# nirschl-lab/stain2stain

Hardware: AMD Instinct MI355X
Metric: paired 256x256 stain tiles/sec (full CFM optimisation step) (higher is better)
Workload: dtype bf16

## Files before the change

stain2stain_amd/csrc/conv3x3_wgrad_mfma.hip:

```cpp
#include "common.h"
#include <stdlib.h>
#include <type_traits>

struct WgradArgs {
  const void* dy;
  const void* x0;
  const void* x1;
  float* part;
  int lddy, Cout, ld0, c0, ld1, c1;
  int B, H, W, tilesY, tilesX, ntiles, S;
  int lgc;
  int lgh, lgw;
  int xcd;
};

namespace {

template <typename T> struct WPiece;
template <> struct WPiece<bf16_t> {
  bf16x8 v;
  __device__ __forceinline__ void zero() {
#pragma unroll
    for (int i = 0; i < 8; ++i) v[i] = (bf16_t)0.0f;
  }
  __device__ __forceinline__ void load(const bf16_t* p) { v = *reinterpret_cast<const bf16x8*>(p); }
  __device__ __forceinline__ void to_lds(char* hi, int, int off) const { *reinterpret_cast<bf16x8*>(hi + off) = v; }
};
template <> struct WPiece<float> {
  f32x4 a, b;
  __device__ __forceinline__ void zero() {
#pragma unroll
    for (int i = 0; i < 4; ++i) { a[i] = 0.f; b[i] = 0.f; }
  }
  __device__ __forceinline__ void load(const float* p) {
    a = *reinterpret_cast<const f32x4*>(p);
    b = *reinterpret_cast<const f32x4*>(p + 4);
  }
  __device__ __forceinline__ void to_lds(char* hi, int img_stride, int off) const {
    bf16x8 h, m, l;
#pragma unroll
    for (int i = 0; i < 8; ++i) {
      const float x = i < 4 ? a[i] : b[i - 4];
      h[i] = (bf16_t)x;
      const float r1 = x - (float)h[i];
      m[i] = (bf16_t)r1;
      l[i] = (bf16_t)(r1 - (float)m[i]);
    }
    *reinterpret_cast<bf16x8*>(hi + off) = h;
    *reinterpret_cast<bf16x8*>(hi + img_stride + off) = m;
    *reinterpret_cast<bf16x8*>(hi + 2 * img_stride + off) = l;
  }
};

typedef __attribute__((address_space(3))) s16x4 lds_s16x4;

__device__ __forceinline__ bf16x8 tr_frag(const char* p_rows0, int row_stride4) {
  s16x4 lo = __builtin_amdgcn_ds_read_tr16_b64_v4i16((lds_s16x4*)(p_rows0));
  s16x4 hi = __builtin_amdgcn_ds_read_tr16_b64_v4i16((lds_s16x4*)(p_rows0 + row_stride4));
  bf16x4 l4 = __builtin_bit_cast(bf16x4, lo), h4 = __builtin_bit_cast(bf16x4, hi);
  bf16x8 r;
#pragma unroll
  for (int i = 0; i < 4; ++i) { r[i] = l4[i]; r[4 + i] = h4[i]; }
  return r;
}

template <typename T, int TH, int TW>
__global__ __launch_bounds__(256, (std::is_same<T, float>::value ? 1 : 2)) void conv3x3_wgrad_kernel(WgradArgs a) {
  constexpr bool SPLIT = std::is_same<T, float>::value;
  constexpr int NIMG = SPLIT ? 3 : 1;
  constexpr int NPX = TH * TW;
  constexpr int HW_ = TW + 2, HALO = (TH + 2) * HW_;
  constexpr int DY_BYTES = 2 * NPX * 64;
  constexpr int X_BYTES = 2 * HALO * 64;
  constexpr int DY_PIECES = NPX * 8, DY_IT = (DY_PIECES + 255) / 256;
  constexpr int X_PIECES = HALO * 8, X_IT = (X_PIECES + 255) / 256;
  constexpr int KSTEPS = NPX / 16;
  static_assert(TW % 16 == 0, "a k-step is 16 consecutive pixels of one tile row");

  extern __shared__ __attribute__((aligned(16))) char smem[];
  char* const ldsDY = smem;
  char* const ldsX = smem + NIMG * DY_BYTES;

  const T* __restrict__ dy = static_cast<const T*>(a.dy);
  const T* __restrict__ x0 = static_cast<const T*>(a.x0);
  const T* __restrict__ x1 = static_cast<const T*>(a.x1);

  const int tid = threadIdx.x, lane = tid & 63, wave = tid >> 6;
  const int wco = wave >> 1, wci = wave & 1;
  const int ci0 = blockIdx.x * 64, co0 = blockIdx.y * 64;
  const int cin = a.c0 + a.c1;

  const int g = lane >> 4, q = (lane & 15) >> 2, p = lane & 3;
  const int frag_off = ((g >> 1) * 8 + q) * 64 + ((g & 1) * 16 + p * 4) * 2;

  f32x16 acc[9];
#pragma unroll
  for (int t = 0; t < 9; ++t)
#pragma unroll
    for (int j = 0; j < 16; ++j) acc[t][j] = 0.f;

  WPiece<T> dreg[DY_IT];
  WPiece<T> xreg[X_IT];

  auto load_tile = [&](int tile) {
    int bt = tile;
    const int tx = bt % a.tilesX; bt /= a.tilesX;
    const int ty = bt % a.tilesY;
    const int img = bt / a.tilesY;
    const int y0 = ty * TH, xs = tx * TW;
#pragma unroll
    for (int i = 0; i < DY_IT; ++i) {
      const int idx = tid + i * 256;
      const int px = idx >> 3, pc = idx & 7;
      const int py = px / TW, pxx = px - py * TW;
      const int gy = y0 + py, gx = xs + pxx, co = co0 + pc * 8;
      dreg[i].zero();
      if (idx < DY_PIECES && gy < a.H && gx < a.W && co < a.Cout)
        dreg[i].load(dy + ((long)(img * a.H + gy) * a.W + gx) * a.lddy + co);
    }
#pragma unroll
    for (int i = 0; i < X_IT; ++i) {
      const int idx = tid + i * 256;
      const int px = idx >> 3, pc = idx & 7;
      const int hy = px / HW_, hx = px - hy * HW_;
      const int gy = y0 - 1 + hy, gx = xs - 1 + hx, ci = ci0 + pc * 8;
      xreg[i].zero();
      if (idx < X_PIECES && gy >= 0 && gy < a.H && gx >= 0 && gx < a.W) {
        const long pix = (long)(img * a.H + gy) * a.W + gx;
        if (ci < a.c0) xreg[i].load(x0 + pix * a.ld0 + ci);
        else if (ci < cin) xreg[i].load(x1 + pix * a.ld1 + (ci - a.c0));
      }
    }
  };
  auto store_tile = [&]() {
#pragma unroll
    for (int i = 0; i < DY_IT; ++i) {
      const int idx = tid + i * 256;
      const int px = idx >> 3, pc = idx & 7;
      if (idx < DY_PIECES)
        dreg[i].to_lds(ldsDY, DY_BYTES, (pc >> 2) * (NPX * 64) + px * 64 + (pc & 3) * 16);
    }
#pragma unroll
    for (int i = 0; i < X_IT; ++i) {
      const int idx = tid + i * 256;
      const int px = idx >> 3, pc = idx & 7;
      if (idx < X_PIECES)
        xreg[i].to_lds(ldsX, X_BYTES, (pc >> 2) * (HALO * 64) + px * 64 + (pc & 3) * 16);
    }
  };

  const char* const Ahi = ldsDY + wco * (NPX * 64) + frag_off;
  const char* const Bhi = ldsX + wci * (HALO * 64) + frag_off;

  int tile = blockIdx.z;
  if (tile < a.ntiles) load_tile(tile);
  for (; tile < a.ntiles; tile += a.S) {
    __syncthreads();
    store_tile();
    __syncthreads();
    if (tile + a.S < a.ntiles) load_tile(tile + a.S);
#pragma unroll
    for (int ks = 0; ks < KSTEPS; ++ks) {
      const int m0 = ks * 16;
      const int py = m0 / TW, px = m0 - py * TW;
      const bf16x8 af = tr_frag(Ahi + m0 * 64, 4 * 64);
      bf16x8 am, al;
      if constexpr (SPLIT) {
        am = tr_frag(Ahi + DY_BYTES + m0 * 64, 4 * 64);
        al = tr_frag(Ahi + 2 * DY_BYTES + m0 * 64, 4 * 64);
      }
#pragma unroll
      for (int tap = 0; tap < 9; ++tap) {
        const int hoff = ((py + tap / 3) * HW_ + px + tap % 3) * 64;
        const bf16x8 bfr = tr_frag(Bhi + hoff, 4 * 64);
        if constexpr (SPLIT) {
          const bf16x8 bm = tr_frag(Bhi + X_BYTES + hoff, 4 * 64);
          const bf16x8 bl = tr_frag(Bhi + 2 * X_BYTES + hoff, 4 * 64);
          acc[tap] = __builtin_amdgcn_mfma_f32_32x32x16_bf16(am, bm, acc[tap], 0, 0, 0);
          acc[tap] = __builtin_amdgcn_mfma_f32_32x32x16_bf16(al, bfr, acc[tap], 0, 0, 0);
          acc[tap] = __builtin_amdgcn_mfma_f32_32x32x16_bf16(af, bl, acc[tap], 0, 0, 0);
          acc[tap] = __builtin_amdgcn_mfma_f32_32x32x16_bf16(am, bfr, acc[tap], 0, 0, 0);
          acc[tap] = __builtin_amdgcn_mfma_f32_32x32x16_bf16(af, bm, acc[tap], 0, 0, 0);
        }
        acc[tap] = __builtin_amdgcn_mfma_f32_32x32x16_bf16(af, bfr, acc[tap], 0, 0, 0);
      }
    }
  }

  const int r = lane & 31, h = lane >> 5;
  const int ci = ci0 + wci * 32 + r;
#pragma unroll
  for (int tap = 0; tap < 9; ++tap) {
#pragma unroll
    for (int j = 0; j < 16; ++j) {
      const int co = co0 + wco * 32 + (j & 3) + 8 * (j >> 2) + 4 * h;
      if (co < a.Cout && ci < cin)
        a.part[(((long)blockIdx.z * 9 + tap) * a.Cout + co) * cin + ci] = acc[tap][j];
    }
  }
}

__device__ __attribute__((aligned(64))) char g_wgrad_zero_page[64];
typedef __attribute__((address_space(3))) void lds_void_t;
typedef __attribute__((address_space(1))) const void gbl_void_t;

__device__ __forceinline__ void dma16_asm(const void* gsrc, unsigned lds_dst) {
  unsigned keep;
  asm volatile("s_mov_b32 %0, m0\n\ts_mov_b32 m0, %2\n\ts_nop 0\n\tglobal_load_lds_dwordx4 %1, off\n\ts_mov_b32 m0, %0"
               : "=&s"(keep) : "v"(gsrc), "s"(lds_dst) : "memory");
}

template <int TH, int TW>
__global__ __launch_bounds__(256, 2) void conv3x3_wgrad_dma_kernel(WgradArgs a) {
  using T = bf16_t;
  constexpr int NW = 4, NT = 9;
  constexpr int NPX = TH * TW;
  constexpr int HW_ = TW + 2, HR = TH + 2, HALO = HR * HW_;
  constexpr int XROWS = (HALO + 31) / 32 * 32;
  constexpr int DY_BYTES = 2 * NPX * 64, X_BYTES = 2 * XROWS * 64;
  constexpr int DYGRP = 2 * NPX / 16, XGRP = 2 * XROWS / 16;
  constexpr int DYG = DYGRP / NW;
  constexpr int XG = XGRP / NW;
  constexpr int BUF = DY_BYTES + X_BYTES;
  constexpr int KSTEPS = NPX / 16;
  static_assert(DYGRP % 4 == 0 && XGRP % 4 == 0, "DMA groups split evenly over 4 waves");

  extern __shared__ __attribute__((aligned(16))) char smem[];
  const T* __restrict__ dy = static_cast<const T*>(a.dy);
  const T* __restrict__ x0 = static_cast<const T*>(a.x0);
  const T* __restrict__ x1 = static_cast<const T*>(a.x1);

  const int tid = threadIdx.x, lane = tid & 63;
  const int wave = __builtin_amdgcn_readfirstlane(tid >> 6);
  const int wco = (wave & 3) >> 1, wci = wave & 1;
  unsigned bx = blockIdx.x, by = blockIdx.y, bz = blockIdx.z;
  if (a.xcd) {
    const unsigned L = bx + gridDim.x * (by + gridDim.y * bz), per = gridDim.x * gridDim.y * gridDim.z / 8;
    unsigned Lq = (L & 7) * per + (L >> 3);
    bx = Lq % gridDim.x; Lq /= gridDim.x;
    by = Lq % gridDim.y; bz = Lq / gridDim.y;
  }
  const int ci0 = bx * 64, co0 = by * 64;
  const int cin = a.c0 + a.c1;
  const int drow = lane >> 2, dslot = lane & 3;
  const int zsplit = (int)bz;

  const int g = lane >> 4, q = (lane & 15) >> 2, p = lane & 3;
  const int frag_off = ((g >> 1) * 8 + q) * 64 + ((g & 1) * 16 + p * 4) * 2;

  f32x16 acc[NT];
#pragma unroll
  for (int t = 0; t < NT; ++t)
#pragma unroll
    for (int j = 0; j < 16; ++j) acc[t][j] = 0.f;

  int dy_off[DYG], dy_py[DYG], dy_px[DYG];
  bool dy_ok[DYG];
#pragma unroll
  for (int j = 0; j < DYG; ++j) {
    const int grp = wave + NW * j;
    const int half = grp / (NPX / 16), px = (grp % (NPX / 16)) * 16 + drow;
    const int co = co0 + half * 32 + dslot * 8;
    dy_py[j] = px / TW; dy_px[j] = px - dy_py[j] * TW;
    dy_ok[j] = co < a.Cout;
    dy_off[j] = (dy_py[j] * a.W + dy_px[j]) * a.lddy + co;
  }
  const T* x_ptr[XG];
  int x_off[XG], x_ld[XG], x_hy[XG], x_hx[XG];
#pragma unroll
  for (int j = 0; j < XG; ++j) {
    const int grp = wave + NW * j;
    const int half = grp / (XROWS / 16), px = (grp % (XROWS / 16)) * 16 + drow;
    const int ci = ci0 + half * 32 + dslot * 8;
    x_hy[j] = px / HW_; x_hx[j] = px - x_hy[j] * HW_;
    x_ptr[j] = nullptr; x_ld[j] = 0;
    if (px < HALO) {
      if (ci < a.c0) { x_ptr[j] = x0 + ci; x_ld[j] = a.ld0; }
      else if (ci < cin) { x_ptr[j] = x1 + (ci - a.c0); x_ld[j] = a.ld1; }
    }
    x_off[j] = ((x_hy[j] - 1) * a.W + (x_hx[j] - 1)) * x_ld[j];
  }

  auto dma_tile = [&](int tile, int buf) {
    int bt = tile;
    const int tx = bt % a.tilesX; bt /= a.tilesX;
    const int ty = bt % a.tilesY;
    const int img = bt / a.tilesY;
    const int y0 = ty * TH, xs = tx * TW;
    const long pixbase = (long)(img * a.H + y0) * a.W + xs;
    const bool interior = y0 >= 1 && y0 + TH + 1 <= a.H && xs >= 1 && xs + TW + 1 <= a.W;
    const unsigned base = (unsigned)(uintptr_t)(__attribute__((address_space(3))) char*)smem + buf * BUF;
    if (interior) {
#pragma unroll
      for (int j = 0; j < DYG; ++j) {
        const void* src = dy_ok[j] ? (const void*)(dy + pixbase * a.lddy + dy_off[j]) : (const void*)g_wgrad_zero_page;
        dma16_asm(src, __builtin_amdgcn_readfirstlane(base + (wave + NW * j) * 1024));
      }
#pragma unroll
      for (int j = 0; j < XG; ++j) {
        const void* src = x_ptr[j] ? (const void*)(x_ptr[j] + pixbase * x_ld[j] + x_off[j]) : (const void*)g_wgrad_zero_page;
        dma16_asm(src, __builtin_amdgcn_readfirstlane(base + DY_BYTES + (wave + NW * j) * 1024));
      }
    } else {
#pragma unroll
      for (int j = 0; j < DYG; ++j) {
        const int gy = y0 + dy_py[j], gx = xs + dy_px[j];
        const void* src = g_wgrad_zero_page;
        if (gy < a.H && gx < a.W && dy_ok[j]) src = dy + pixbase * a.lddy + dy_off[j];
        dma16_asm(src, __builtin_amdgcn_readfirstlane(base + (wave + NW * j) * 1024));
      }
#pragma unroll
      for (int j = 0; j < XG; ++j) {
        const int gy = y0 - 1 + x_hy[j], gx = xs - 1 + x_hx[j];
        const void* src = g_wgrad_zero_page;
        if (x_ptr[j] && gy >= 0 && gy < a.H && gx >= 0 && gx < a.W) src = x_ptr[j] + pixbase * x_ld[j] + x_off[j];
        dma16_asm(src, __builtin_amdgcn_readfirstlane(base + DY_BYTES + (wave + NW * j) * 1024));
      }
    }
  };

  int tile = zsplit;
  int buf = 0;
  if (tile < a.ntiles) dma_tile(tile, 0);
  asm volatile("s_waitcnt vmcnt(0)" ::: "memory");
  __builtin_amdgcn_s_barrier();
  for (; tile < a.ntiles; tile += a.S) {
    if (tile + a.S < a.ntiles) dma_tile(tile + a.S, buf ^ 1);
    const char* const Ahi = smem + buf * BUF + wco * (NPX * 64) + frag_off;
    const char* const Bhi = smem + buf * BUF + DY_BYTES + wci * (XROWS * 64) + frag_off;
#pragma unroll
    for (int ks = 0; ks < KSTEPS; ++ks) {
      const int m0 = ks * 16;
      const int py = m0 / TW, px = m0 - py * TW;
      const bf16x8 af = tr_frag(Ahi + m0 * 64, 4 * 64);
#pragma unroll
      for (int t = 0; t < NT; ++t) {
        const int hoff = ((py + t / 3) * HW_ + px + t % 3) * 64;
        const bf16x8 bfr = tr_frag(Bhi + hoff, 4 * 64);
        acc[t] = __builtin_amdgcn_mfma_f32_32x32x16_bf16(af, bfr, acc[t], 0, 0, 0);
      }
    }
    __builtin_amdgcn_sched_barrier(0);
    asm volatile("s_waitcnt vmcnt(0)" ::: "memory");
    __builtin_amdgcn_s_barrier();
    buf ^= 1;
  }

  const int r = lane & 31, h = lane >> 5;
  const int ci = ci0 + wci * 32 + r;
#pragma unroll
  for (int t = 0; t < NT; ++t) {
#pragma unroll
    for (int j = 0; j < 16; ++j) {
      const int co = co0 + wco * 32 + (j & 3) + 8 * (j >> 2) + 4 * h;
      if (co < a.Cout && ci < cin)
        a.part[(((long)zsplit * 9 + t) * a.Cout + co) * cin + ci] = acc[t][j];
    }
  }
}

template <int ZG>
__global__ __launch_bounds__(64 * ZG) void wgrad_reduce_kernel(const float* __restrict__ part, float* __restrict__ grad, int S, int Cout,
                                    int Cin, int accumulate) {
  __shared__ float tile[ZG][9][65];
  const long n = (long)Cout * Cin;
  const int il = threadIdx.x & 63, zg = threadIdx.x >> 6;
  const long i = (long)blockIdx.x * 64 + il;
  float s[9];
#pragma unroll
  for (int t = 0; t < 9; ++t) s[t] = 0.f;
  if (i < n) {
    for (int z = zg; z < S; z += ZG)
#pragma unroll
      for (int t = 0; t < 9; ++t) s[t] += part[((long)z * 9 + t) * n + i];
  }
#pragma unroll
  for (int t = 0; t < 9; ++t) tile[zg][t][il] = s[t];
  __syncthreads();
  const long base = (long)blockIdx.x * 64 * 9;
  for (int k = threadIdx.x; k < 576; k += 64 * ZG) {
    const long o = base + k;
    if (o < n * 9) {
      const int t = k % 9, j = k / 9;
      float v = 0.f;
#pragma unroll
      for (int g = 0; g < ZG; g += 4) v += (tile[g][t][j] + tile[g + 1][t][j]) + (tile[g + 2][t][j] + tile[g + 3][t][j]);
      grad[o] = accumulate ? grad[o] + v : v;
    }
  }
}

template <typename T, int TH, int TW>
int launch_wgrad(WgradArgs& a, hipStream_t s) {
  constexpr int NIMG = std::is_same<T, float>::value ? 3 : 1;
  constexpr int lds = NIMG * (2 * TH * TW * 64 + 2 * (TH + 2) * (TW + 2) * 64);
  a.tilesY = cdiv(a.H, TH);
  a.tilesX = cdiv(a.W, TW);
  a.ntiles = a.B * a.tilesY * a.tilesX;
  if (a.S > a.ntiles) return S2S_ERR_SHAPE;
  auto kern = conv3x3_wgrad_kernel<T, TH, TW>;
  static unsigned long long attr_devs = 0;
  if (int rc = s2s_allow_dyn_lds(reinterpret_cast<const void*>(kern), lds, &attr_devs)) return rc;
  dim3 grid(cdiv(a.c0 + a.c1, 64), cdiv(a.Cout, 64), a.S);
  hipLaunchKernelGGL(kern, grid, dim3(256), lds, s, a);
  S2S_LAUNCH_CHECK();
  return S2S_OK;
}

template <int TH, int TW>
int launch_wgrad_dma(WgradArgs& a, hipStream_t s) {
  constexpr int XROWS = ((TH + 2) * (TW + 2) + 31) / 32 * 32;
  constexpr int lds = 2 * (2 * TH * TW * 64 + 2 * XROWS * 64);
  a.tilesY = cdiv(a.H, TH);
  a.tilesX = cdiv(a.W, TW);
  a.ntiles = a.B * a.tilesY * a.tilesX;
  if (a.S > a.ntiles) return S2S_ERR_SHAPE;
  auto kern = conv3x3_wgrad_dma_kernel<TH, TW>;
  static unsigned long long attr_devs = 0;
  if (int rc = s2s_allow_dyn_lds(reinterpret_cast<const void*>(kern), lds, &attr_devs)) return rc;
  dim3 grid(cdiv(a.c0 + a.c1, 64), cdiv(a.Cout, 64), a.S);
  static const int xcd_aware = [] { const char* e = getenv("S2S_WGRAD_XCD"); return e ? atoi(e) : 1; }();
  a.xcd = xcd_aware && ((long)grid.x * grid.y * grid.z) % 8 == 0;
  hipLaunchKernelGGL(kern, grid, dim3(256), lds, s, a);
  S2S_LAUNCH_CHECK();
  return S2S_OK;
}

template <int TH, int TW, bool S2D = false>
__global__ __launch_bounds__(256, 2) void conv2x2_wgrad_dma_kernel(WgradArgs a) {
  using T = bf16_t;
  constexpr int NT = 4;
  constexpr int NPX = TH * TW;
  constexpr int HW_ = TW + 1, HR = TH + 1, HALO = HR * HW_;
  constexpr int XROWS = (HALO + 31) / 32 * 32;
  constexpr int DY_BYTES = 2 * NPX * 64, X_BYTES = 2 * XROWS * 64;
  constexpr int DYG = 2 * NPX / 16 / 4;
  constexpr int XG = 2 * XROWS / 16 / 4;
  constexpr int BUF = DY_BYTES + X_BYTES;
  constexpr int KSTEPS = NPX / 16;
  static_assert((2 * NPX / 16) % 4 == 0 && (2 * XROWS / 16) % 4 == 0, "DMA groups split evenly over 4 waves");

  extern __shared__ __attribute__((aligned(16))) char smem[];
  const T* __restrict__ dy = static_cast<const T*>(a.dy);
  const T* __restrict__ x0 = static_cast<const T*>(a.x0);

  const int tid = threadIdx.x, lane = tid & 63;
  const int wave = __builtin_amdgcn_readfirstlane(tid >> 6);
  const int wco = wave >> 1, wci = wave & 1;
  const int ci0 = blockIdx.x * 64, co0 = blockIdx.y * 64;
  const int cin = a.c0;
  const int Hi = a.H + 1, Wi = a.W + 1;
  const int drow = lane >> 2, dslot = lane & 3;
  const int zsplit = (int)blockIdx.z;

  const int g = lane >> 4, q = (lane & 15) >> 2, p = lane & 3;
  const int frag_off = ((g >> 1) * 8 + q) * 64 + ((g & 1) * 16 + p * 4) * 2;

  f32x16 acc[NT];
#pragma unroll
  for (int t = 0; t < NT; ++t)
#pragma unroll
    for (int j = 0; j < 16; ++j) acc[t][j] = 0.f;

  int dy_off[DYG], dy_py[DYG], dy_px[DYG];
  bool dy_ok[DYG];
#pragma unroll
  for (int j = 0; j < DYG; ++j) {
    const int grp = wave + 4 * j;
    const int half = grp / (NPX / 16), px = (grp % (NPX / 16)) * 16 + drow;
    const int co = co0 + half * 32 + dslot * 8;
    dy_py[j] = px / TW; dy_px[j] = px - dy_py[j] * TW;
    dy_ok[j] = co < a.Cout;
    dy_off[j] = (dy_py[j] * a.W + dy_px[j]) * a.lddy + co;
  }
  const T* x_ptr[XG];
  int x_off[XG], x_hy[XG], x_hx[XG];
#pragma unroll
  for (int j = 0; j < XG; ++j) {
    const int grp = wave + 4 * j;
    const int half = grp / (XROWS / 16), px = (grp % (XROWS / 16)) * 16 + drow;
    const int ci = ci0 + half * 32 + dslot * 8;
    x_hy[j] = px / HW_; x_hx[j] = px - x_hy[j] * HW_;
    if (S2D) {
      const int rs = ci >> a.lgc;
      x_ptr[j] = (px < HALO && ci < cin) ? x0 + (ci & ((1 << a.lgc) - 1)) : nullptr;
      x_hy[j] = 2 * x_hy[j] + (rs >> 1) - 1;
      x_hx[j] = 2 * x_hx[j] + (rs & 1) - 1;
      x_off[j] = 0;
    } else {
      x_ptr[j] = (px < HALO && ci < cin) ? x0 + ci : nullptr;
      x_off[j] = (x_hy[j] * Wi + x_hx[j]) * a.ld0;
    }
  }

  auto dma_tile = [&](int tile, int buf) {
    int bt = tile;
    const int tx = bt % a.tilesX; bt /= a.tilesX;
    const int ty = bt % a.tilesY;
    const int img = bt / a.tilesY;
    const int y0 = ty * TH, xs = tx * TW;
    const long pixbase = (long)(img * a.H + y0) * a.W + xs;
    const long xbase = (long)(img * Hi + y0) * Wi + xs;
    const bool interior = !S2D && y0 + TH <= a.H && xs + TW <= a.W;
    const unsigned base = (unsigned)(uintptr_t)(__attribute__((address_space(3))) char*)smem + buf * BUF;
    if (interior) {
#pragma unroll
      for (int j = 0; j < DYG; ++j) {
        const void* src = dy_ok[j] ? (const void*)(dy + pixbase * a.lddy + dy_off[j]) : (const void*)g_wgrad_zero_page;
        dma16_asm(src, __builtin_amdgcn_readfirstlane(base + (wave + 4 * j) * 1024));
      }
#pragma unroll
      for (int j = 0; j < XG; ++j) {
        const void* src = x_ptr[j] ? (const void*)(x_ptr[j] + xbase * a.ld0 + x_off[j]) : (const void*)g_wgrad_zero_page;
        dma16_asm(src, __builtin_amdgcn_readfirstlane(base + DY_BYTES + (wave + 4 * j) * 1024));
      }
    } else {
#pragma unroll
      for (int j = 0; j < DYG; ++j) {
        const int gy = y0 + dy_py[j], gx = xs + dy_px[j];
        const void* src = g_wgrad_zero_page;
        if (gy < a.H && gx < a.W && dy_ok[j]) src = dy + pixbase * a.lddy + dy_off[j];
        dma16_asm(src, __builtin_amdgcn_readfirstlane(base + (wave + 4 * j) * 1024));
      }
#pragma unroll
      for (int j = 0; j < XG; ++j) {
        const void* src = g_wgrad_zero_page;
        if (S2D) {
          const int py = 2 * y0 + x_hy[j], px = 2 * xs + x_hx[j];
          if (x_ptr[j] && (unsigned)py < (unsigned)(2 * a.H) && (unsigned)px < (unsigned)(2 * a.W))
            src = x_ptr[j] + ((long)(img * 2 * a.H + py) * (2 * a.W) + px) * a.ld0;
        } else {
          const int gy = y0 + x_hy[j], gx = xs + x_hx[j];
          if (x_ptr[j] && gy < Hi && gx < Wi) src = x_ptr[j] + xbase * a.ld0 + x_off[j];
        }
        dma16_asm(src, __builtin_amdgcn_readfirstlane(base + DY_BYTES + (wave + 4 * j) * 1024));
      }
    }
  };

  int tile = zsplit;
  int buf = 0;
  if (tile < a.ntiles) dma_tile(tile, 0);
  asm volatile("s_waitcnt vmcnt(0)" ::: "memory");
  __builtin_amdgcn_s_barrier();
  for (; tile < a.ntiles; tile += a.S) {
    if (tile + a.S < a.ntiles) dma_tile(tile + a.S, buf ^ 1);
    const char* const Ahi = smem + buf * BUF + wco * (NPX * 64) + frag_off;
    const char* const Bhi = smem + buf * BUF + DY_BYTES + wci * (XROWS * 64) + frag_off;
#pragma unroll
    for (int ks = 0; ks < KSTEPS; ++ks) {
      const int m0 = ks * 16;
      const int py = m0 / TW, px = m0 - py * TW;
      const bf16x8 af = tr_frag(Ahi + m0 * 64, 4 * 64);
#pragma unroll
      for (int t = 0; t < NT; ++t) {
        const int hoff = ((py + t / 2) * HW_ + px + t % 2) * 64;
        const bf16x8 bfr = tr_frag(Bhi + hoff, 4 * 64);
        acc[t] = __builtin_amdgcn_mfma_f32_32x32x16_bf16(af, bfr, acc[t], 0, 0, 0);
      }
    }
    __builtin_amdgcn_sched_barrier(0);
    asm volatile("s_waitcnt vmcnt(0)" ::: "memory");
    __builtin_amdgcn_s_barrier();
    buf ^= 1;
  }

  const int r = lane & 31, h = lane >> 5;
  const int ci = ci0 + wci * 32 + r;
#pragma unroll
  for (int t = 0; t < NT; ++t) {
#pragma unroll
    for (int j = 0; j < 16; ++j) {
      const int co = co0 + wco * 32 + (j & 3) + 8 * (j >> 2) + 4 * h;
      if (co < a.Cout && ci < cin)
        a.part[(((long)zsplit * NT + t) * a.Cout + co) * cin + ci] = acc[t][j];
    }
  }
}

__global__ __launch_bounds__(256, 1) void conv2x2_wgrad_flat_kernel(WgradArgs a) {
  using T = bf16_t;
  constexpr int NT = 4, NPX = 128;
  constexpr int DY_BYTES = 2 * NPX * 64, PLANE = NPX * 64, X_BYTES = 2 * NT * PLANE;
  constexpr int DYG = 2 * NPX / 16 / 4;
  constexpr int XG = 2 * NT * NPX / 16 / 4;
  constexpr int KSTEPS = NPX / 16;

  extern __shared__ __attribute__((aligned(16))) char smem[];
  const T* __restrict__ dy = static_cast<const T*>(a.dy);
  const T* __restrict__ x0 = static_cast<const T*>(a.x0);
  const int tid = threadIdx.x, lane = tid & 63;
  const int wave = __builtin_amdgcn_readfirstlane(tid >> 6);
  const int wco = wave >> 1, wci = wave & 1;
  const int ci0 = blockIdx.x * 64, co0 = blockIdx.y * 64;
  const int cin = a.c0;
  const int h = 1 << a.lgh, w = 1 << a.lgw;
  const int npix = a.B << (a.lgh + a.lgw);
  const int drow = lane >> 2, dslot = lane & 3;
  const int zsplit = (int)blockIdx.z;
  const int g = lane >> 4, q = (lane & 15) >> 2, p4 = lane & 3;
  const int frag_off = ((g >> 1) * 8 + q) * 64 + ((g & 1) * 16 + p4 * 4) * 2;

  f32x16 acc[NT];
#pragma unroll
  for (int t = 0; t < NT; ++t)
#pragma unroll
    for (int j = 0; j < 16; ++j) acc[t][j] = 0.f;

  auto dma_tile = [&](int tile) {
    const int p0 = tile * NPX;
    const unsigned base = (unsigned)(uintptr_t)(__attribute__((address_space(3))) char*)smem;
#pragma unroll
    for (int j = 0; j < DYG; ++j) {
      const int grp = wave + 4 * j;
      const int half = grp / (NPX / 16), m = (grp % (NPX / 16)) * 16 + drow;
      const int co = co0 + half * 32 + dslot * 8, p = p0 + m;
      const void* src = g_wgrad_zero_page;
      if (p < npix && co < a.Cout) src = dy + (long)p * a.lddy + co;
      dma16_asm(src, __builtin_amdgcn_readfirstlane(base + grp * 1024));
    }
#pragma unroll
    for (int j = 0; j < XG; ++j) {
      const int grp = wave + 4 * j;
      const int half = grp >> 5, tap = (grp >> 3) & 3, m = (grp & 7) * 16 + drow;
      const int ci = ci0 + half * 32 + dslot * 8, p = p0 + m;
      const void* src = g_wgrad_zero_page;
      if (p < npix && ci < cin) {
        const int n = p >> (a.lgh + a.lgw), iy = (p >> a.lgw) & (h - 1), ix = p & (w - 1);
        const int rs = ci >> a.lgc, cc = ci & ((1 << a.lgc) - 1);
        const int py = 2 * (iy + (tap >> 1)) + (rs >> 1) - 1, px = 2 * (ix + (tap & 1)) + (rs & 1) - 1;
        if ((unsigned)py < (unsigned)(2 * h) && (unsigned)px < (unsigned)(2 * w))
          src = x0 + ((long)(n * 2 * h + py) * (2 * w) + px) * a.ld0 + cc;
      }
      dma16_asm(src, __builtin_amdgcn_readfirstlane(base + DY_BYTES + grp * 1024));
    }
  };

  for (int tile = zsplit; tile < a.ntiles; tile += a.S) {
    dma_tile(tile);
    asm volatile("s_waitcnt vmcnt(0)" ::: "memory");
    __builtin_amdgcn_s_barrier();
    const char* const Ahi = smem + wco * (NPX * 64) + frag_off;
    const char* const Bhi = smem + DY_BYTES + wci * (NT * PLANE) + frag_off;
#pragma unroll
    for (int ks = 0; ks < KSTEPS; ++ks) {
      const int m0 = ks * 16;
      const bf16x8 af = tr_frag(Ahi + m0 * 64, 4 * 64);
#pragma unroll
      for (int t = 0; t < NT; ++t) {
        const bf16x8 bfr = tr_frag(Bhi + t * PLANE + m0 * 64, 4 * 64);
        acc[t] = __builtin_amdgcn_mfma_f32_32x32x16_bf16(af, bfr, acc[t], 0, 0, 0);
      }
    }
    __builtin_amdgcn_sched_barrier(0);
    asm volatile("s_waitcnt lgkmcnt(0)" ::: "memory");
    __builtin_amdgcn_s_barrier();
  }
  const int r = lane & 31, hh = lane >> 5;
  const int ci = ci0 + wci * 32 + r;
#pragma unroll
  for (int t = 0; t < NT; ++t) {
#pragma unroll
    for (int j = 0; j < 16; ++j) {
      const int co = co0 + wco * 32 + (j & 3) + 8 * (j >> 2) + 4 * hh;
      if (co < a.Cout && ci < cin) a.part[(((long)zsplit * NT + t) * a.Cout + co) * cin + ci] = acc[t][j];
    }
  }
}

__global__ __launch_bounds__(256, 2) void conv2x2_wgrad_small_kernel(WgradArgs a, float* __restrict__ grad, int accumulate) {
  using T = bf16_t;
  constexpr int NT = 4, NPX = 128;
  constexpr int DY_BYTES = 2 * NPX * 64, PLANE = NPX * 64, X_BYTES = 2 * NT * PLANE, BUF = DY_BYTES + X_BYTES;
  constexpr int DYG = 2 * NPX / 16 / 4;
  constexpr int XG = 2 * NT * NPX / 16 / 4;
  constexpr int KSTEPS = NPX / 16;

  extern __shared__ __attribute__((aligned(16))) char smem[];
  const T* __restrict__ dy = static_cast<const T*>(a.dy);
  const T* __restrict__ x0 = static_cast<const T*>(a.x0);
  const int tid = threadIdx.x, lane = tid & 63;
  const int wave = __builtin_amdgcn_readfirstlane(tid >> 6);
  const int wco = wave >> 1, wci = wave & 1;
  const int c0 = blockIdx.x * 16, co0 = blockIdx.y * 64;
  const int C = a.c0 >> 2;
  const int h = 1 << a.lgh, w = 1 << a.lgw;
  const int npix = a.B << (a.lgh + a.lgw);
  const int drow = lane >> 2, dslot = lane & 3;
  const int g = lane >> 4, q = (lane & 15) >> 2, p4 = lane & 3;
  const int frag_off = ((g >> 1) * 8 + q) * 64 + ((g & 1) * 16 + p4 * 4) * 2;

  f32x16 acc[NT];
#pragma unroll
  for (int t = 0; t < NT; ++t)
#pragma unroll
    for (int j = 0; j < 16; ++j) acc[t][j] = 0.f;

  auto dma_tile = [&](int tile, int buf) {
    const int p0 = tile * NPX;
    const unsigned base = (unsigned)(uintptr_t)(__attribute__((address_space(3))) char*)smem + buf * BUF;
#pragma unroll
    for (int j = 0; j < DYG; ++j) {
      const int grp = wave + 4 * j;
      const int half = grp / (NPX / 16), m = (grp % (NPX / 16)) * 16 + drow;
      const int co = co0 + half * 32 + dslot * 8, p = p0 + m;
      const void* src = g_wgrad_zero_page;
      if (p < npix && co < a.Cout) src = dy + (long)p * a.lddy + co;
      dma16_asm(src, __builtin_amdgcn_readfirstlane(base + grp * 1024));
    }
#pragma unroll
    for (int j = 0; j < XG; ++j) {
      const int grp = wave + 4 * j;
      const int half = grp >> 5, tap = (grp >> 3) & 3, m = (grp & 7) * 16 + drow;
      const int vci = half * 32 + dslot * 8, rs = vci >> 4, cc = c0 + (vci & 15), p = p0 + m;
      const void* src = g_wgrad_zero_page;
      if (p < npix && cc < C) {
        const int n = p >> (a.lgh + a.lgw), iy = (p >> a.lgw) & (h - 1), ix = p & (w - 1);
        const int py = 2 * (iy + (tap >> 1)) + (rs >> 1) - 1, px = 2 * (ix + (tap & 1)) + (rs & 1) - 1;
        if ((unsigned)py < (unsigned)(2 * h) && (unsigned)px < (unsigned)(2 * w))
          src = x0 + ((long)(n * 2 * h + py) * (2 * w) + px) * a.ld0 + cc;
      }
      dma16_asm(src, __builtin_amdgcn_readfirstlane(base + DY_BYTES + grp * 1024));
// ... 623 lines not shown
```

Measured before the change: 2262.

## Use buffer-load LDS DMA with OOB zeroing and interleave prefetch with MFMA k-steps

Swaps global_load_lds plus a zero-page pointer select for buffer_load...lds with per-tile buffer resource descriptors, so out-of-bounds halo and channel lanes are zero-filled by hardware range checking instead of branchy address selection. The next tile's DMA pieces are now spread across the k-step loop, two per step, instead of being issued in one burst before compute. Halo B fragments are reused across k-steps through a rolling 3x3 register window, which cuts repeated LDS transposed reads. It adds a shape guard on the descriptor's record range, a MIXED template variant for concat inputs whose split is not 32-aligned, and ablation variants behind a compile flag.

```diff
diff --git a/stain2stain_amd/csrc/conv3x3_wgrad_mfma.hip b/stain2stain_amd/csrc/conv3x3_wgrad_mfma.hip
--- a/stain2stain_amd/csrc/conv3x3_wgrad_mfma.hip
+++ b/stain2stain_amd/csrc/conv3x3_wgrad_mfma.hip
@@ -1,6 +1,7 @@
 #include "common.h"
 #include <stdlib.h>
 #include <type_traits>
+
 
 struct WgradArgs {
   const void* dy;
@@ -210,9 +211,25 @@
                : "=&s"(keep) : "v"(gsrc), "s"(lds_dst) : "memory");
 }
 
-template <int TH, int TW>
+typedef __attribute__((ext_vector_type(4))) int i32x4;
+constexpr unsigned WG_RECORDS = 0x80000000u;
+constexpr unsigned WG_OOB = 0xffffff00u;
+__device__ __forceinline__ i32x4 wgrad_rsrc(uintptr_t base) {
+  i32x4 r;
+  r[0] = __builtin_amdgcn_readfirstlane((int)(unsigned)base);
+  r[1] = __builtin_amdgcn_readfirstlane((int)((base >> 32) & 0xffff));
+  r[2] = (int)WG_RECORDS;
+  r[3] = 0x00020000;
+  return r;
+}
+__device__ __forceinline__ void dma16_buf(const i32x4& rsrc, unsigned voff, unsigned lds_dst) {
+  unsigned keep;
+  asm volatile("s_mov_b32 %0, m0\n\ts_mov_b32 m0, %3\n\ts_nop 0\n\tbuffer_load_dwordx4 %1, %2, 0 offen lds\n\ts_mov_b32 m0, %0"
+               : "=&s"(keep) : "v"(voff), "s"(rsrc), "s"(lds_dst));
+}
+
+template <int TH, int TW, bool MIXED, int ABL>
 __global__ __launch_bounds__(256, 2) void conv3x3_wgrad_dma_kernel(WgradArgs a) {
-  using T = bf16_t;
   constexpr int NW = 4, NT = 9;
   constexpr int NPX = TH * TW;
   constexpr int HW_ = TW + 2, HR = TH + 2, HALO = HR * HW_;
@@ -221,15 +238,15 @@
   constexpr int DYGRP = 2 * NPX / 16, XGRP = 2 * XROWS / 16;
   constexpr int DYG = DYGRP / NW;
   constexpr int XG = XGRP / NW;
+  constexpr int NP = DYG + XG;
   constexpr int BUF = DY_BYTES + X_BYTES;
   constexpr int KSTEPS = NPX / 16;
   static_assert(DYGRP % 4 == 0 && XGRP % 4 == 0, "DMA groups split evenly over 4 waves");
+  constexpr int PK = (NP + 1) / 2;
+  static_assert(PK < KSTEPS, "pieces land before the tile-end wait");
+  static_assert(TW == 16, "a k-step is one tile row");
 
   extern __shared__ __attribute__((aligned(16))) char smem[];
-  const T* __restrict__ dy = static_cast<const T*>(a.dy);
-  const T* __restrict__ x0 = static_cast<const T*>(a.x0);
-  const T* __restrict__ x1 = static_cast<const T*>(a.x1);
-
   const int tid = threadIdx.x, lane = tid & 63;
   const int wave = __builtin_amdgcn_readfirstlane(tid >> 6);
   const int wco = (wave & 3) >> 1, wci = wave & 1;
@@ -254,96 +271,114 @@
 #pragma unroll
     for (int j = 0; j < 16; ++j) acc[t][j] = 0.f;
 
-  int dy_off[DYG], dy_py[DYG], dy_px[DYG];
-  bool dy_ok[DYG];
+  unsigned dy_voff[DYG];
+  int dy_py[DYG], dy_px[DYG];
 #pragma unroll
   for (int j = 0; j < DYG; ++j) {
     const int grp = wave + NW * j;
     const int half = grp / (NPX / 16), px = (grp % (NPX / 16)) * 16 + drow;
     const int co = co0 + half * 32 + dslot * 8;
     dy_py[j] = px / TW; dy_px[j] = px - dy_py[j] * TW;
-    dy_ok[j] = co < a.Cout;
-    dy_off[j] = (dy_py[j] * a.W + dy_px[j]) * a.lddy + co;
-  }
-  const T* x_ptr[XG];
-  int x_off[XG], x_ld[XG], x_hy[XG], x_hx[XG];
+    dy_voff[j] = co < a.Cout ? (unsigned)(((dy_py[j] * a.W + dy_px[j]) * a.lddy + co) * 2) : WG_OOB;
+  }
+  unsigned x_voff[XG];
+  int x_hy[XG], x_hx[XG], x_mode[XG];
+  bool x_hi[XG];
 #pragma unroll
   for (int j = 0; j < XG; ++j) {
     const int grp = wave + NW * j;
     const int half = grp / (XROWS / 16), px = (grp % (XROWS / 16)) * 16 + drow;
-    const int ci = ci0 + half * 32 + dslot * 8;
+    const int cbase = ci0 + half * 32, ci = cbase + dslot * 8;
     x_hy[j] = px / HW_; x_hx[j] = px - x_hy[j] * HW_;
-    x_ptr[j] = nullptr; x_ld[j] = 0;
-    if (px < HALO) {
-      if (ci < a.c0) { x_ptr[j] = x0 + ci; x_ld[j] = a.ld0; }
-      else if (ci < cin) { x_ptr[j] = x1 + (ci - a.c0); x_ld[j] = a.ld1; }
-    }
-    x_off[j] = ((x_hy[j] - 1) * a.W + (x_hx[j] - 1)) * x_ld[j];
-  }
-
-  auto dma_tile = [&](int tile, int buf) {
+    x_mode[j] = __builtin_amdgcn_readfirstlane(cbase + 32 <= a.c0 || a.c1 == 0 ? 0 : cbase >= a.c0 ? 1 : 2);
+    x_hi[j] = ci >= a.c0;
+    const int ld = x_hi[j] ? a.ld1 : a.ld0, ch = x_hi[j] ? ci - a.c0 : ci;
+    x_voff[j] = px < HALO && ci < cin ? (unsigned)(((x_hy[j] * a.W + x_hx[j]) * ld + ch) * 2) : WG_OOB;
+  }
+
+  struct TileSrc {
+    i32x4 rdy, rx0, rx1;
+    int limy, limx, sy, sx;
+  };
+  auto tile_src = [&](int tile) {
     int bt = tile;
     const int tx = bt % a.tilesX; bt /= a.tilesX;
     const int ty = bt % a.tilesY;
     const int img = bt / a.tilesY;
     const int y0 = ty * TH, xs = tx * TW;
-    const long pixbase = (long)(img * a.H + y0) * a.W + xs;
-    const bool interior = y0 >= 1 && y0 + TH + 1 <= a.H && xs >= 1 && xs + TW + 1 <= a.W;
-    const unsigned base = (unsigned)(uintptr_t)(__attribute__((address_space(3))) char*)smem + buf * BUF;
-    if (interior) {
-#pragma unroll
-      for (int j = 0; j < DYG; ++j) {
-        const void* src = dy_ok[j] ? (const void*)(dy + pixbase * a.lddy + dy_off[j]) : (const void*)g_wgrad_zero_page;
-        dma16_asm(src, __builtin_amdgcn_readfirstlane(base + (wave + NW * j) * 1024));
-      }
-#pragma unroll
-      for (int j = 0; j < XG; ++j) {
-        const void* src = x_ptr[j] ? (const void*)(x_ptr[j] + pixbase * x_ld[j] + x_off[j]) : (const void*)g_wgrad_zero_page;
-        dma16_asm(src, __builtin_amdgcn_readfirstlane(base + DY_BYTES + (wave + NW * j) * 1024));
-      }
+    const long pix = (long)(img * a.H + y0) * a.W + xs;
+    const long hpix = pix - a.W - 1;
+    TileSrc s;
+    s.rdy = wgrad_rsrc((uintptr_t)a.dy + (uintptr_t)(pix * a.lddy * 2));
+    s.rx0 = wgrad_rsrc((uintptr_t)a.x0 + (uintptr_t)(hpix * a.ld0 * 2));
+    s.rx1 = wgrad_rsrc((uintptr_t)a.x1 + (uintptr_t)(hpix * a.ld1 * 2));
+    s.limy = a.H - y0; s.limx = a.W - xs;
+    s.sy = y0 - 1; s.sx = xs - 1;
+    return s;
+  };
+  auto dma_piece = [&](const TileSrc& s, int i, unsigned base) {
+    if (ABL & 1) return;
+    if (i < DYG) {
+      const unsigned v = dy_py[i] < s.limy && dy_px[i] < s.limx ? dy_voff[i] : WG_OOB;
+      dma16_buf(s.rdy, v, base + (wave + NW * i) * 1024);
     } else {
-#pragma unroll
-      for (int j = 0; j < DYG; ++j) {
-        const int gy = y0 + dy_py[j], gx = xs + dy_px[j];
-        const void* src = g_wgrad_zero_page;
-        if (gy < a.H && gx < a.W && dy_ok[j]) src = dy + pixbase * a.lddy + dy_off[j];
-        dma16_asm(src, __builtin_amdgcn_readfirstlane(base + (wave + NW * j) * 1024));
-      }
-#pragma unroll
-      for (int j = 0; j < XG; ++j) {
-        const int gy = y0 - 1 + x_hy[j], gx = xs - 1 + x_hx[j];
-        const void* src = g_wgrad_zero_page;
-        if (x_ptr[j] && gy >= 0 && gy < a.H && gx >= 0 && gx < a.W) src = x_ptr[j] + pixbase * x_ld[j] + x_off[j];
-        dma16_asm(src, __builtin_amdgcn_readfirstlane(base + DY_BYTES + (wave + NW * j) * 1024));
+      const int j = i - DYG;
+      const unsigned v = (unsigned)(x_hy[j] + s.sy) < (unsigned)a.H && (unsigned)(x_hx[j] + s.sx) < (unsigned)a.W ? x_voff[j] : WG_OOB;
+      const unsigned dst = base + DY_BYTES + (wave + NW * j) * 1024;
+      if (!MIXED || x_mode[j] != 2) {
+        i32x4 r = s.rx0;
+        if (x_mode[j] == 1) { r[0] = s.rx1[0]; r[1] = s.rx1[1]; }
+        dma16_buf(r, v, dst);
+      } else if (x_hi[j]) {
+        dma16_buf(s.rx1, v, dst);
+      } else {
+        dma16_buf(s.rx0, v, dst);
       }
     }
   };
+  const unsigned lds0 = (unsigned)(uintptr_t)(__attribute__((address_space(3))) char*)smem;
 
   int tile = zsplit;
-  int buf = 0;
-  if (tile < a.ntiles) dma_tile(tile, 0);
+  {
+    const TileSrc s = tile_src(tile);
+#pragma unroll
+    for (int i = 0; i < NP; ++i) dma_piece(s, i, lds0);
+  }
   asm volatile("s_waitcnt vmcnt(0)" ::: "memory");
   __builtin_amdgcn_s_barrier();
+
+  int cur = 0;
   for (; tile < a.ntiles; tile += a.S) {
-    if (tile + a.S < a.ntiles) dma_tile(tile + a.S, buf ^ 1);
-    const char* const Ahi = smem + buf * BUF + wco * (NPX * 64) + frag_off;
-    const char* const Bhi = smem + buf * BUF + DY_BYTES + wci * (XROWS * 64) + frag_off;
+    const bool pf = tile + a.S < a.ntiles;
+    TileSrc s = tile_src(pf ? tile + a.S : tile);
+    if (!pf) { s.limy = 0; s.sy = -(1 << 30); }
+    const unsigned pbase = lds0 + (cur ^ 1) * BUF;
+    const char* const Ahi = smem + cur * BUF + wco * (NPX * 64) + frag_off;
+    const char* const Bhi = smem + cur * BUF + DY_BYTES + wci * (XROWS * 64) + frag_off;
+    bf16x8 hf[3][3];
 #pragma unroll
     for (int ks = 0; ks < KSTEPS; ++ks) {
-      const int m0 = ks * 16;
-      const int py = m0 / TW, px = m0 - py * TW;
-      const bf16x8 af = tr_frag(Ahi + m0 * 64, 4 * 64);
-#pragma unroll
-      for (int t = 0; t < NT; ++t) {
-        const int hoff = ((py + t / 3) * HW_ + px + t % 3) * 64;
-        const bf16x8 bfr = tr_frag(Bhi + hoff, 4 * 64);
-        acc[t] = __builtin_amdgcn_mfma_f32_32x32x16_bf16(af, bfr, acc[t], 0, 0, 0);
-      }
+      bf16x8 af;
+      if (!(ABL & 2)) {
+        af = tr_frag(Ahi + ks * 16 * 64, 4 * 64);
+#pragma unroll
+        for (int kh = (ks == 0 ? 0 : 2); kh < 3; ++kh)
+#pragma unroll
+          for (int kw = 0; kw < 3; ++kw) hf[(ks + kh) % 3][kw] = tr_frag(Bhi + ((ks + kh) * HW_ + kw) * 64, 4 * 64);
+      }
+#pragma unroll
+      for (int i = 2 * ks; i < 2 * ks + 2 && i < NP; ++i) dma_piece(s, i, pbase);
+      if (ABL & 2) continue;
+#pragma unroll
+      for (int t = 0; t < NT; ++t)
+        acc[t] = __builtin_amdgcn_mfma_f32_32x32x16_bf16(af, hf[(ks + t / 3) % 3][t % 3], acc[t], 0, 0, 0);
     }
     __builtin_amdgcn_sched_barrier(0);
-    asm volatile("s_waitcnt vmcnt(0)" ::: "memory");
-    __builtin_amdgcn_s_barrier();
-    buf ^= 1;
+    if (!(ABL & 4)) {
+      asm volatile("s_waitcnt vmcnt(0)" ::: "memory");
+      __builtin_amdgcn_s_barrier();
+    }
+    cur ^= 1;
   }
 
   const int r = lane & 31, h = lane >> 5;
@@ -415,9 +450,26 @@
   a.tilesX = cdiv(a.W, TW);
   a.ntiles = a.B * a.tilesY * a.tilesX;
   if (a.S > a.ntiles) return S2S_ERR_SHAPE;
-  auto kern = conv3x3_wgrad_dma_kernel<TH, TW>;
-  static unsigned long long attr_devs = 0;
-  if (int rc = s2s_allow_dyn_lds(reinterpret_cast<const void*>(kern), lds, &attr_devs)) return rc;
+  const long ldmax = a.lddy > a.ld0 ? (a.lddy > a.ld1 ? a.lddy : a.ld1) : (a.ld0 > a.ld1 ? a.ld0 : a.ld1);
+  if ((long)(TH + 2) * (a.W + 1) * ldmax * 2 >= (long)WG_RECORDS) return S2S_ERR_SHAPE;
+  const bool mixed = a.c1 > 0 && a.c0 % 32 != 0;
+  int variant = mixed ? 1 : 0;
+  void (*kern)(WgradArgs) = mixed ? conv3x3_wgrad_dma_kernel<TH, TW, true, 0> : conv3x3_wgrad_dma_kernel<TH, TW, false, 0>;
+#ifdef S2S_ABLATE
+  static const int dbg = [] { const char* e = getenv("S2S_WGRAD_DBG"); return e ? atoi(e) : 0; }();
+  if (dbg && !mixed) {
+    switch (dbg) {
+      case 1: kern = conv3x3_wgrad_dma_kernel<TH, TW, false, 1>; break;
+      case 2: kern = conv3x3_wgrad_dma_kernel<TH, TW, false, 2>; break;
+      case 4: kern = conv3x3_wgrad_dma_kernel<TH, TW, false, 4>; break;
+      case 5: kern = conv3x3_wgrad_dma_kernel<TH, TW, false, 5>; break;
+      default: return S2S_ERR_SHAPE;
+    }
+    variant = 2;
+  }
+#endif
+  static unsigned long long attr_devs[3] = {};
+  if (int rc = s2s_allow_dyn_lds(reinterpret_cast<const void*>(kern), lds, &attr_devs[variant])) return rc;
   dim3 grid(cdiv(a.c0 + a.c1, 64), cdiv(a.Cout, 64), a.S);
   static const int xcd_aware = [] { const char* e = getenv("S2S_WGRAD_XCD"); return e ? atoi(e) : 1; }();
   a.xcd = xcd_aware && ((long)grid.x * grid.y * grid.z) % 8 == 0;
```

After: 2273 (median of 6 runs). Within noise of the previous version (+0.5%).
